# paolomandica/HALO

Measured on AMD Instinct MI355X. Metric: acquisition-scored images/sec (1024x2048, C=256, 19 cls), higher is better.
Workload: dtype f64

## Files before the change

halo_amd/_lib.py:

```python
import ctypes as C
import os
import threading

from . import _build

F32, F64 = 0, 1
I64, I32, U8 = 2, 3, 4
F16, BF16 = 5, 6
UNC = {"entropy": 0, "pixel_entropy": 1, "oracle_acc": 2}
UNC_ZEROS = 3
PUR = {"ripu": 0, "oracle_ripu": 1, "hyper": 2, "none": 3, "radius": 4, "euc_norm": 5}
E_UNSUPPORTED = -2
SELECT = {"auto": 0, "serial": 1, "binned": 2}
LOSS_CE, LOSS_NL = 1, 2
SWEEP_REASONS = ("done", "bad_values", "bin_overflow", "survivors", "exhausted", "not_run")
PAD = {"zeros": 0, "reflect": 1, "replicate": 2, "circular": 3}
FLAG_NORMALIZE = 1
WINDOW = {"box": 0, "hist": 1}
WINDOW_ROUTES = ("generic", "tile3", "tiled")


def score_flags(normalize, padding_mode="zeros"):
    return (FLAG_NORMALIZE if normalize else 0) | (PAD[padding_mode] << 8)

# ... 101 lines not shown
    "halo_sgd_plan": (_int, [C.POINTER(_i64), _i64, C.POINTER(_i64), C.POINTER(_i64), C.POINTER(_i64)]),
    "halo_sgd_step": (_int, [C.POINTER(SgdArgs), _vp]),
    "halo_event_create": (_vp, []),
    "halo_event_record": (_int, [_vp, _vp]),
    "halo_event_elapsed_ms": (_int, [_vp, _vp, C.POINTER(C.c_float)]),
    "halo_event_destroy": (_int, [_vp]),
    "halo_pack_pick_tables": (_int, [_vp, _vp, _i64, _i64, _vp, _i64, _vp]),
    "halo_reset_round_state": (_int, [_vp, _vp, _vp, _i64, _vp]),
    "halo_undo_picks": (_int, [_vp, _vp, _i64, _i64, _i64, _i64, _i64, _i64, _vp, _vp, _vp, _vp]),
    "halo_device_identity": (_int, [_int, C.c_char_p, _sz]),
    "halo_select_workspace_bytes": (_sz, [_i64, _i64, _i64, _i64, _i64]),
    "halo_score_range_bytes": (_sz, [_i64]),
    "halo_score_range": (_int, [_vp, _int, _i64, _i64, _i64, _vp, _vp]),
    "halo_greedy_select": (_int, [_vp, _int, _i64, _i64, _i64, _i64, _i64, _i64, _vp, _vp, _vp, _vp, _vp, _vp,
                                  _vp, _sz, _int, _vp, _vp, _vp]),
}

ABI_VERSION = 13

_lock = threading.Lock()
_handle = None


class HaloHipError(RuntimeError):
    pass


class HaloUnsupported(HaloHipError):
    """The kernel declined this configuration (HALO_E_UNSUPPORTED); the caller may take another HIP route."""

# ... 136 lines not shown
```

halo_amd/core/active/build.py:

```python
import math
import os
import struct
import zlib

import numpy as np
import torch
from PIL import Image

from ... import _lib
from ..configs import cfg
from ..utils.hyperbolic import HyperMapper, bilinear_align_corners
from .floating_region import FloatingRegionScore, new_score_range, score_maps, score_maps_lowres, _workspace


def greedy_select(score, n_regions, active_radius, mask_radius, active, selected, active_mask, ground_truth,
                  return_picks=True, method=None, out=None, score_range=None, handover=None):
    dev = _lib.require_device(score, active, selected, active_mask, ground_truth)
    B, H, W = score.shape
    for t in (score, active, selected, active_mask, ground_truth):
        assert t.shape == (B, H, W) and t.is_contiguous(), "greedy_select expects contiguous (B,H,W) tensors"
    assert active.dtype == torch.bool and selected.dtype == torch.bool
    assert active_mask.dtype == torch.int64 and ground_truth.dtype == torch.int64
    n = int(max(0, min(int(n_regions), H * W)))
    picks = n_picked = None
    if out is not None:
        picks, n_picked = out
        assert picks.shape == (B, max(n, 1), 3) and picks.dtype == torch.float64 and picks.is_contiguous() and picks.device == dev
        assert n_picked.shape == (B,) and n_picked.dtype == torch.int32 and n_picked.is_contiguous() and n_picked.device == dev
        return_picks = True
    elif return_picks:
        picks = torch.zeros((B, max(n, 1), 3), dtype=torch.float64, device=dev)
        n_picked = torch.zeros((B,), dtype=torch.int32, device=dev)
    if handover is not None:
        assert handover.shape == (B, 2) and handover.dtype == torch.int32 and handover.is_contiguous() and handover.device == dev
    if n == 0 or B == 0:
        if handover is not None:
            handover.zero_()
        return (picks[:, :0], n_picked) if return_picks else None
    L = _lib.lib()
    name = method or os.environ.get("HALO_SELECT", "auto")
    if name not in _lib.SELECT:
        raise ValueError("greedy_select: method must be one of %s, got %r" % (sorted(_lib.SELECT), name))
    method = _lib.SELECT[name]
    nws = L.halo_select_workspace_bytes(B, H, W, n, int(mask_radius)) if method != _lib.SELECT["serial"] else 256
    ws = _workspace(dev, nws, "select")
    if score_range is not None:
        assert score_range.is_contiguous() and score_range.device == dev and score_range.numel() >= L.halo_score_range_bytes(B)
    rc = L.halo_greedy_select(_lib.ptr(score), _lib.dtype_code(score), B, H, W, n, int(active_radius),
                              int(mask_radius), _lib.ptr(active), _lib.ptr(selected), _lib.ptr(active_mask),
                              _lib.ptr(ground_truth), _lib.ptr(picks), _lib.ptr(n_picked), _lib.ptr(ws), ws.numel(),
                              method, _lib.ptr(score_range), _lib.ptr(handover), _lib.stream_ptr(dev))
    _lib.check(rc, "halo_greedy_select")
    return (picks, n_picked) if return_picks else None


def _stage(t, dev, dtype):
    if t.device == dev and t.dtype == dtype and t.is_contiguous():
        return t, False
    return t.to(device=dev, dtype=dtype).contiguous(), True


def select_pixels_to_label(score, active_regions, active_radius, mask_radius, active, selected, active_mask,
                           ground_truth):
    dev = _lib.require_device(score)
    assert score.dim() == 2, "score must be (H, W)"
    sc, sc_c = _stage(score, dev, score.dtype if score.dtype in (torch.float32, torch.float64) else torch.float32)
    ac, ac_c = _stage(active, dev, torch.bool)
# ... 648 lines not shown
```

halo_amd/csrc/halo_select.hip:

```cpp
#include "halo_select_common.hpp"

namespace halo {

constexpr int SEL_TPB_MAIN = 512;
constexpr int SEL_TPB_RESUME = 256;

struct SelGeom { int H, W, th_shift, tw_shift, nty, ntx, nt; };

template <typename T, int TSH, int TSW>
__device__ __forceinline__ Cand tile_reduce(const T *__restrict__ sc, const SelGeom &g, int ty, int tx, int lane,
                                            int wy0, int wy1, int wx0, int wx1, int py0 = 1, int py1 = 0, int px0 = 1,
                                            int px1 = 0)
{
    constexpr int TW = 1 << TSW, NPL = (1 << (TSH + TSW)) / 64;
    static_assert(NPL >= 1, "tile smaller than a wave");
    const int x0 = tx << TSW, y0 = ty << TSH;
    double v[NPL];
#pragma unroll
    for (int i = 0; i < NPL; ++i) {
        const int e = lane + 64 * i;
        const int y = y0 + (e >> TSW), x = x0 + (e & (TW - 1));
        const int yc = y < g.H ? y : g.H - 1, xc = x < g.W ? x : g.W - 1;
        v[i] = (double)sc[(size_t)yc * g.W + xc];
    }
// ... 195 lines not shown
static bool serial_supported(int64_t H, int64_t W)
{
    if (H > 65535 || W > 65535) return false;
    const SelGeom g = make_geom(H, W);
    return (size_t)g.nt * 12 <= 96 * 1024;
}

extern "C" size_t halo_select_workspace_bytes(int64_t B, int64_t H, int64_t W, int64_t n_regions, int64_t mask_radius)
{
    if (B <= 0 || H <= 0 || W <= 0) return 0;
    if (n_regions > H * W) n_regions = H * W;
    const BinPlan p = binned_plan(B, H, W, n_regions, 0, mask_radius);
    return p.ok ? p.total_bytes + 256 : 256;
}

template <typename T, int A, int B_, int EPT>
static int launch_serial(const SelGeom &g, size_t lds, dim3 grid, hipStream_t st, void *score, int n_regions, int arad, int mrad,
                         uint8_t *active, uint8_t *selected, int64_t *active_mask, const int64_t *gt, double *picks,
                         int32_t *n_picked, const SelHdr *resume, int n_images)
{
    static LdsLimitSeen seen;
    if (lds > 64 * 1024 && !raise_lds_limit(seen, (const void *)k_greedy_select<T, A, B_, EPT>, 128 * 1024))
        return fail(HALO_E_LAUNCH, "halo_greedy_select: cannot raise the dynamic LDS limit");
    hipLaunchKernelGGL((k_greedy_select<T, A, B_, EPT>), grid, dim3(SEL_TPB_MAIN), lds, st, (T *)score, g, n_regions, arad, mrad, active,
                       selected, (long long *)active_mask, (const long long *)gt, picks, n_picked, resume, n_images);
    return HALO_OK;
}

template <typename T, int A, int B_, int EPT>
static int launch_resume(const SelGeom &g, size_t lds, dim3 grid, hipStream_t st, void *score, int n_regions, int arad, int mrad,
// ... 102 lines not shown
```

halo_amd/csrc/halo_select_binned.hip:

```cpp
#include <stdlib.h>
#include <string.h>

#include "halo_select_plan.hpp"

namespace halo {

constexpr int SW_TPB = 256;
constexpr int SW_SURV = 256;
constexpr int FWIN = 1024;

constexpr int BIN_CAP = 128;
constexpr int PL_U = 8;
constexpr int SW_MB = 4;

struct BinWs {
    SelHdr *hdr;
    SelHdr *rng;
    const unsigned *rng_hist;
    unsigned *hist1, *cbase, *cm;
    unsigned *fcur;
    unsigned long long *ckey;
    unsigned *cpos;
    unsigned long long *okmin_inv, *okmax;
    unsigned *plist;
// ... 75 lines not shown
            const unsigned long long k = order_key(v[u]);
            if (k < KEY_POS_INF && k != KEY_NEG_INF) {
                double t;
                atomicAdd(&h[coarse_bin(v[u], r, t)], 1u);
            }
        }
    }
    __syncthreads();
    unsigned *g = ws.hist1 + (size_t)b * NB1;
    for (int j = threadIdx.x; j < NB1; j += 256)
        if (h[j]) atomicAdd(&g[j], h[j]);
}

__global__ void __launch_bounds__(256) k_sel_scan1(BinWs ws, BinGeom g)
{
    __shared__ unsigned sc_c[256], sc_m[256], s_t1;
    const int b = blockIdx.x, tid = threadIdx.x;
    SelHdr *hdr = ws.hdr + b;
    const ValRange r = sel_range(ws.rng[b]);
    const bool ext = ws.rng_hist && (ws.rng[b].flags & SEL_F_HIST);
    const unsigned *hist = (ext ? ws.rng_hist : ws.hist1) + (size_t)b * NB1;
    unsigned c[8], m[8], tc = 0, tm = 0;
#pragma unroll
    for (int i = 0; i < 8; ++i) {
        c[i] = r.ok ? hist[tid * 8 + i] : 0u;
        m[i] = (c[i] + g.target - 1) / g.target;
        tc += c[i];
        tm += m[i];
    }
    sc_c[tid] = tc;
    sc_m[tid] = tm;
    if (tid == 0) s_t1 = 0;
    __syncthreads();
    for (int d = 1; d < 256; d <<= 1) {
        const unsigned ac = tid + d < 256 ? sc_c[tid + d] : 0u, am = tid + d < 256 ? sc_m[tid + d] : 0u;
        __syncthreads();
        sc_c[tid] += ac;
        sc_m[tid] += am;
        __syncthreads();
    }
    unsigned above_c = tid + 1 < 256 ? sc_c[tid + 1] : 0u, above_m = tid + 1 < 256 ? sc_m[tid + 1] : 0u;
    unsigned S[8], M[8];
#pragma unroll
    for (int i = 7; i >= 0; --i) {
        M[i] = above_m;
        above_c += c[i];
        above_m += m[i];
        S[i] = above_c;
    }
    int mine = -1;
#pragma unroll
    for (int i = 0; i < 8; ++i)
        if (S[i] >= g.kneed) mine = tid * 8 + i;
    if (mine > 0) atomicMax(&s_t1, (unsigned)mine);
    unsigned *cb = ws.cbase + (size_t)b * NB1, *cmm = ws.cm + (size_t)b * NB1;
#pragma unroll
    for (int i = 0; i < 8; ++i) { cb[tid * 8 + i] = M[i]; cmm[tid * 8 + i] = m[i]; }
    __syncthreads();
    unsigned t1 = s_t1;
    if ((int)(t1 >> 3) == tid) {
        const int i = t1 & 7;
        unsigned trunc = 0, nf;
        unsigned s_here = 0, m_here = 0, M_here = 0;
#pragma unroll
        for (int q = 0; q < 8; ++q)
            if (q == i) { s_here = S[q]; m_here = m[q]; M_here = M[q]; }
        if (!r.ok) { t1 = NB1; trunc = 1; nf = 0; }
        else if (s_here > g.captot) { t1 += 1; trunc = 1; nf = M_here; }
        else nf = M_here + m_here;
        if (ext && t1 > 0) trunc = 1;
        hdr->t1 = t1;
        hdr->truncated = trunc;
        hdr->nf = nf;
    }
    __syncthreads();
    if (ext && tid == 0) ws.rng[b].flags &= ~(unsigned)SEL_F_HIST;
}

template <typename T>
__global__ void __launch_bounds__(256) k_sel_place(const T *__restrict__ score, BinWs ws, BinGeom g)
{
    __shared__ unsigned s_base[NB1], s_m[NB1];
    const int b = blockIdx.y, tid = threadIdx.x;
    SelHdr *hdr = ws.hdr + b;
    const ValRange r = sel_range(ws.rng[b]);
    const unsigned t1 = hdr->t1;
    if (!r.ok || t1 >= NB1) return;
    for (int j = tid; j < NB1; j += 256) { s_base[j] = ws.cbase[(size_t)b * NB1 + j]; s_m[j] = ws.cm[(size_t)b * NB1 + j]; }
    __syncthreads();
    const T *sc = score + (size_t)b * g.H * g.W;
    unsigned *fcur = ws.fcur + (size_t)b * g.nfmax;
    unsigned long long *ckey = ws.ckey + (size_t)b * g.nfmax * BIN_CAP;
    unsigned *cpos = ws.cpos + (size_t)b * g.nfmax * BIN_CAP;
    bool overflow = false;
    for (int y = blockIdx.x; y < g.H; y += gridDim.x)
        for (int x0 = 0; x0 < g.W; x0 += PL_U * 256) {
            double v[PL_U];
#pragma unroll
            for (int u = 0; u < PL_U; ++u) {
                const int x = x0 + u * 256 + tid;
                v[u] = x < g.W ? (double)sc[(size_t)y * g.W + x] : __longlong_as_double(0xfff0000000000000ll);
            }
            unsigned long long k[PL_U];
            unsigned f[PL_U], slot[PL_U];
            bool cand[PL_U];
#pragma unroll
            for (int u = 0; u < PL_U; ++u) {
                k[u] = order_key(v[u]);
                cand[u] = k[u] < KEY_POS_INF && k[u] != KEY_NEG_INF;
                double t = 0.0;
                const int j = cand[u] ? coarse_bin(v[u], r, t) : 0;
                cand[u] = cand[u] && (unsigned)j >= t1;
                f[u] = 0;
                if (cand[u]) {
                    const unsigned mj = s_m[j];
                    unsigned sb = (unsigned)((t - (double)j) * (double)mj);
                    sb = sb > mj - 1 ? mj - 1 : sb;
                    f[u] = s_base[j] + (mj - 1 - sb);
                }
            }
            unsigned long long cm[PL_U];
            unsigned f_first = 0u, tot = 0u;
            cm[0] = __ballot(cand[0]);
            bool uni = __builtin_popcountll(cm[0]) >= 32;
            if (uni) {
                f_first = (unsigned)__builtin_amdgcn_readlane((int)f[0], (int)__builtin_ctzll(cm[0]));
                tot = (unsigned)__builtin_popcountll(cm[0]);
// ... 17 lines not shown
            }
#pragma unroll
            for (int u = 0; u < PL_U; ++u)
                if (cand[u]) {
                    if (slot[u] < (unsigned)BIN_CAP) {
                        const size_t sl = (size_t)f[u] * BIN_CAP + slot[u];
                        ckey[sl] = k[u];
                        cpos[sl] = ((unsigned)(x0 + u * 256 + tid) << 16) | (unsigned)y;
                    } else overflow = true;
                }
        }
    if (__any(overflow) && (tid & 63) == 0) atomicOr(&hdr->flags, (unsigned)SEL_F_OVERFLOW);
}

template <typename T>
__global__ void __launch_bounds__(256) k_sel_full_extrema(const T *__restrict__ score, BinWs ws, BinGeom g)
{
    __shared__ unsigned s_base[NB1], s_m[NB1];
    const int b = blockIdx.y, tid = threadIdx.x;
    const SelHdr *hdr = ws.hdr + b;
    if (!(hdr->flags & SEL_F_OVERFLOW)) return;
    const ValRange r = sel_range(ws.rng[b]);
    const unsigned t1 = hdr->t1;
    if (!r.ok || t1 >= NB1) return;
    for (int j = tid; j < NB1; j += 256) { s_base[j] = ws.cbase[(size_t)b * NB1 + j]; s_m[j] = ws.cm[(size_t)b * NB1 + j]; }
    __syncthreads();
    const T *sc = score + (size_t)b * g.H * g.W;
    const unsigned *fcur = ws.fcur + (size_t)b * g.nfmax;
    unsigned long long *okmin_inv = ws.okmin_inv + (size_t)b * g.nfmax, *okmax = ws.okmax + (size_t)b * g.nfmax;
    for (int y = blockIdx.x; y < g.H; y += gridDim.x)
        for (int x0 = 0; x0 < g.W; x0 += 256) {
            const int x = x0 + tid;
            const double v = x < g.W ? (double)sc[(size_t)y * g.W + x] : __longlong_as_double(0xfff0000000000000ll);
            const unsigned long long k = order_key(v);
            bool cand = k < KEY_POS_INF && k != KEY_NEG_INF;
            double t = 0.0;
            const int j = cand ? coarse_bin(v, r, t) : 0;
            cand = cand && (unsigned)j >= t1;
            unsigned f = 0;
            if (cand) {
                const unsigned mj = s_m[j];
                unsigned sb = (unsigned)((t - (double)j) * (double)mj);
                sb = sb > mj - 1 ? mj - 1 : sb;
                f = s_base[j] + (mj - 1 - sb);
            }
            const bool full = cand && fcur[f] > (unsigned)BIN_CAP;
            unsigned long long todo = __ballot(full);
            while (todo) {
                const int l0 = (int)__builtin_ctzll(todo);
                const unsigned f0 = (unsigned)__builtin_amdgcn_readlane((int)f, l0);
                const bool mine = full && f == f0;
                const unsigned long long kx = wave_max_u64(mine ? k : 0ull), kn = wave_max_u64(mine ? ~k : 0ull);
                if ((tid & 63) == l0) { atomicMax(&okmax[f0], kx); atomicMax(&okmin_inv[f0], kn); }
// ... 94 lines not shown
        if (__ballot(undecided) == 0ull) break;
    }
    const bool is_pick = alive && ((pickm >> lane) & 1ull) != 0ull;
    const int idx = np + (int)__builtin_popcountll(before & pickm);
    if (is_pick && idx < g.n_regions) {
        plist[idx] = pos;
        const int pcx = (int)__umulhi((unsigned)x, g.cmul), pcy = (int)__umulhi((unsigned)y, g.cmul);
        grid[(pcy + 1) * g.gstride + pcx + 1] = (unsigned char)(1 + (((y - pcy * cs) << 4) | (x - pcx * cs)));
    }
    np += (int)__builtin_popcountll(pickm);
    if (np >= g.n_regions) { np = g.n_regions; return 1; }
    return 0;
}

__global__ void __launch_bounds__(SW_TPB, 5) k_sel_sweep(BinWs ws, BinGeom g, int *__restrict__ n_picked, const void *__restrict__ score_maps,
                                                      int score_f64)
{
    extern __shared__ __attribute__((aligned(16))) unsigned char smem[];
    unsigned char *grid = smem;
    unsigned *gridw = reinterpret_cast<unsigned *>(smem);
    unsigned long long *skey = reinterpret_cast<unsigned long long *>(smem + g.grid_bytes);
    unsigned *spos = reinterpret_cast<unsigned *>(skey + SW_SURV);
    unsigned *fwin = spos + SW_SURV;
    unsigned *ctl = fwin + FWIN + 1;

    __builtin_amdgcn_s_setprio(3);
    const int b = blockIdx.x, tid = threadIdx.x, lane = tid & 63, wave = tid >> 6;
    SelHdr *hdr = ws.hdr + b;
    const unsigned nf = hdr->nf;
    const bool truncated = hdr->truncated != 0;
    const unsigned *fcnt = ws.fcur + (size_t)b * g.nfmax;
    const unsigned long long *ckey = ws.ckey + (size_t)b * g.nfmax * BIN_CAP;
    const unsigned *cpos = ws.cpos + (size_t)b * g.nfmax * BIN_CAP;
    unsigned *plist = ws.plist + (size_t)b * g.n_regions;
    const unsigned long long *okmin_inv = ws.okmin_inv + (size_t)b * g.nfmax, *okmax = ws.okmax + (size_t)b * g.nfmax;
    const double *map64 = score_f64 ? (const double *)score_maps + (size_t)b * g.H * g.W : nullptr;
    const float *map32 = score_f64 ? nullptr : (const float *)score_maps + (size_t)b * g.H * g.W;

    for (unsigned i = tid * 16; i < g.grid_bytes; i += SW_TPB * 16) *reinterpret_cast<uint4 *>(smem + i) = make_uint4(0, 0, 0, 0);
    if (tid == 0) { ctl[0] = 0; ctl[1] = 0; }
    __syncthreads();

    int np = 0;
    int fin = 0;
    int why = HALO_SWEEP_DONE;
    const int r = g.mrad, cs = g.cs;

    struct Chunk { unsigned start[SW_MB], cnt[SW_MB], total; bool last, valid, plateau; unsigned pbin; };
    unsigned fw0 = 0, fwn = 0;
    unsigned it_f = 0;
    auto next_chunk = [&]() {
        Chunk c;
#pragma unroll
        for (int i = 0; i < SW_MB; ++i) { c.start[i] = 0; c.cnt[i] = 0; }
        c.total = 0; c.last = true; c.valid = false; c.plateau = false; c.pbin = 0;
        int nb = 0;
        while (it_f < nf) {
            if (fwn == 0 || it_f >= fw0 + fwn) {
                lds_barrier();
                fw0 = it_f;
                fwn = nf - it_f < (unsigned)FWIN ? nf - it_f : (unsigned)FWIN;
                for (unsigned i = tid; i < fwn; i += SW_TPB) fwin[i] = fcnt[fw0 + i];
                __syncthreads();
            }
            const unsigned n = fwin[it_f - fw0];
// ... 150 lines not shown
            if (fin) break;
            knext = wave_max_u64(knext);
            lds_barrier();
            if (lane == 0) skey[wave] = knext;
            lds_barrier();
            knext = skey[0];
#pragma unroll
            for (int i = 1; i < SW_TPB / 64; ++i) knext = skey[i] > knext ? skey[i] : knext;
            lds_barrier();
            if (knext == 0ull) break;
            K = knext;
        }
    };
    auto step = [&](const Chunk &c, const Regs &d) {
        if (c.plateau) { plateau_scan(c.pbin); return; }
        push((unsigned)tid < c.total && grid_alive(d.pos), d.key, d.pos);
        if (!c.last) return;
        resolve_listed();
    };
    Chunk c0 = next_chunk(), c1, c2;
    Regs d0, d1, d2;
    issue(c0, d0);
    c1 = next_chunk(); issue(c1, d1);
    c2 = next_chunk(); issue(c2, d2);
    while (true) {
        if (!c0.valid || fin) break;
        step(c0, d0);
        c0 = next_chunk(); issue(c0, d0);
        if (!c1.valid || fin) break;
        step(c1, d1);
        c1 = next_chunk(); issue(c1, d1);
        if (!c2.valid || fin) break;
        step(c2, d2);
        c2 = next_chunk(); issue(c2, d2);
    }
#ifdef HALO_SWEEP_STAMPS
    if (tid == 0) {
        hdr->pad[0] = (unsigned)(t_f >> 4); hdr->pad[1] = (unsigned)(t_a >> 4); hdr->pad[2] = (unsigned)(t_r >> 4); hdr->pad[3] = (unsigned)(t_b >> 4);
        hdr->nvalid = (unsigned)nb; hdr->ncand = (unsigned)t_surv; hdr->flags = (unsigned)t_smax;
    }
#endif
    if (tid == 0) {
        if (fin == 0) {
            fin = truncated ? 2 : 1;
            if (truncated) why = hdr->t1 >= (unsigned)NB1 ? HALO_SWEEP_BAD_VALUES : HALO_SWEEP_EXHAUSTED;
        }
        if (ws.handover) { ws.handover[2 * b] = fin == 1 ? HALO_SWEEP_DONE : why; ws.handover[2 * b + 1] = np; }
        hdr->np = np;
        hdr->status = fin == 1 ? SEL_DONE : SEL_BAIL;
        if (fin == 1 && n_picked) n_picked[b] = np;
    }
}

constexpr int APPLY_WGS = 32;

template <typename T>
__global__ void __launch_bounds__(256) k_sel_apply(T *__restrict__ score, unsigned char *__restrict__ active,
                                                   unsigned char *__restrict__ selected, long long *__restrict__ active_mask,
                                                   const long long *__restrict__ gt, double *__restrict__ picks, BinWs ws, BinGeom g)
{
    const int b = blockIdx.y, lane = threadIdx.x & 63;
    const int np = ws.hdr[b].np;
    const size_t hw = (size_t)g.H * g.W;
    T *sc = score + (size_t)b * hw;
    unsigned char *act = active + (size_t)b * hw, *sel = selected + (size_t)b * hw;
// ... 21 lines not shown
        const int aw = ax1 - ax0 + 1, an = aw * (ay1 - ay0 + 1);
        const int mw = mx1 - mx0 + 1, mn = mw * (my1 - my0 + 1);
        for (int e = lane; e < an; e += 64) {
            const size_t o = (size_t)(ay0 + e / aw) * g.W + (ax0 + e % aw);
            sel[o] = 1;
            am[o] = gtb[o];
        }
        for (int e = lane; e < mn; e += 64) {
            const size_t o = (size_t)(my0 + e / mw) * g.W + (mx0 + e % mw);
            sc[o] = neg_inf;
            act[o] = 1;
        }
    }
}

}

using namespace halo;

namespace halo {

BinPlan binned_plan(int64_t B, int64_t H, int64_t W, int64_t n_regions, int64_t arad, int64_t mrad)
{
    BinPlan p;
    memset(&p, 0, sizeof(p));
    if (B <= 0 || H <= 0 || W <= 0 || n_regions <= 0 || H > 65535 || W > 65535 || mrad < 1 || mrad > 14) return p;
    BinGeom &g = p.g;
    g.H = (int)H; g.W = (int)W; g.n_regions = (int)n_regions; g.arad = (int)arad; g.mrad = (int)mrad;
    g.cs = (int)mrad + 1;
    g.gcy = (int)cdiv(H, g.cs);
    g.gcx = (int)cdiv(W, g.cs);
    g.gstride = (int)align_up((size_t)g.gcx + 2, 4);
    g.cmul = (unsigned)((0x100000000ull + (unsigned)g.cs - 1) / (unsigned)g.cs);
    g.grid_bytes = (unsigned)align_up((size_t)(g.gcy + 2) * g.gstride + 8, 16);
    p.lds_bytes = g.grid_bytes + (size_t)SW_SURV * 12 + (FWIN + 1) * 4 + 16;
    if (p.lds_bytes > 156 * 1024) return p;
    const unsigned long long hw = (unsigned long long)H * W, win = (unsigned long long)(2 * mrad + 1) * (2 * mrad + 1);
    const unsigned long long kneed = win * (unsigned long long)n_regions < hw ? win * (unsigned long long)n_regions : hw;
    unsigned long long cap = 2 * kneed < 65536 ? 65536 : 2 * kneed;
    if (cap > hw) cap = hw;
    g.kneed = (unsigned)kneed;
    g.captot = (unsigned)cap;
    g.target = (unsigned)(BIN_CAP / 2);
    g.nfmax = (unsigned)(cap / g.target + NB1 + 1);
    size_t o = 0;
    auto take = [&](size_t per_image) { const size_t at = o; o += align_up(per_image * (size_t)B, 256); return at; };
    p.off_hdr = take(sizeof(SelHdr));
    p.off_hist1 = take((size_t)NB1 * 4);
    p.off_fcur = take((size_t)g.nfmax * 4);
    p.off_okmin = take((size_t)g.nfmax * 8);
    p.off_okmax = take((size_t)g.nfmax * 8);
    p.zero_bytes = o;
    p.off_cbase = take((size_t)NB1 * 4);
    p.off_cm = take((size_t)NB1 * 4);
    p.off_ckey = take((size_t)g.nfmax * BIN_CAP * 8);
    p.off_cpos = take((size_t)g.nfmax * BIN_CAP * 4);
// ... 12 lines not shown
    ws.rng = ws.hdr;
    const unsigned gx = (unsigned)(cdiv(hw, 256) < 128 ? cdiv(hw, 256) : 128);
    if (dtype == HALO_F64) hipLaunchKernelGGL(k_sel_range<double>, dim3(gx, (unsigned)B), dim3(256), 0, st, (const double *)score, (long long)hw, ws);
    else hipLaunchKernelGGL(k_sel_range<float>, dim3(gx, (unsigned)B), dim3(256), 0, st, (const float *)score, (long long)hw, ws);
    return HALO_OK;
}

int binned_select(void *score, int dtype, int64_t B, const BinPlan &p, uint8_t *active, uint8_t *selected, int64_t *active_mask,
                  const int64_t *gt, double *picks, int32_t *n_picked, void *workspace, size_t workspace_bytes, hipStream_t st,
                  SelHdr **hdr_out, const void *score_range, int32_t *handover)
{
    if (!workspace || workspace_bytes < p.total_bytes) return fail(HALO_E_WORKSPACE, "halo_greedy_select: workspace too small");
    char *base = (char *)(((uintptr_t)workspace + 255) & ~(uintptr_t)255);
    if ((size_t)(base - (char *)workspace) + p.total_bytes - 256 > workspace_bytes) return fail(HALO_E_WORKSPACE, "halo_greedy_select: workspace too small");
    BinWs ws;
    ws.hdr = (SelHdr *)(base + p.off_hdr);
    ws.rng = score_range ? (SelHdr *)score_range : ws.hdr;
    ws.rng_hist = score_range ? (const unsigned *)((const char *)score_range + range_hist_offset(B)) : nullptr;
    ws.hist1 = (unsigned *)(base + p.off_hist1);
    ws.fcur = (unsigned *)(base + p.off_fcur);
    ws.okmin_inv = (unsigned long long *)(base + p.off_okmin);
    ws.okmax = (unsigned long long *)(base + p.off_okmax);
    ws.cbase = (unsigned *)(base + p.off_cbase);
    ws.cm = (unsigned *)(base + p.off_cm);
    ws.ckey = (unsigned long long *)(base + p.off_ckey);
    ws.cpos = (unsigned *)(base + p.off_cpos);
    ws.plist = (unsigned *)(base + p.off_plist);
    ws.handover = handover;
    const BinGeom &g = p.g;
    const long long hw = (long long)g.H * g.W;
// ... 1 lines not shown
        const size_t n16 = p.zero_bytes / 16;
        const unsigned gz = (unsigned)(cdiv((int64_t)n16, 256) < 512 ? cdiv((int64_t)n16, 256) : 512);
        hipLaunchKernelGGL(k_sel_zero, dim3(gz ? gz : 1u), dim3(256), 0, st, (uint4 *)base, n16);
    }
    const unsigned gx = (unsigned)(cdiv(hw, 256) < 128 ? cdiv(hw, 256) : 128);
    const unsigned gy = (unsigned)(g.H < 128 ? g.H : 128);
    dim3 blk(256);
    if (dtype == HALO_F64) {
        if (!score_range) hipLaunchKernelGGL(k_sel_range<double>, dim3(gx, (unsigned)B), blk, 0, st, (const double *)score, hw, ws);
        hipLaunchKernelGGL(k_sel_hist1<double>, dim3(gx, (unsigned)B), blk, 0, st, (const double *)score, hw, ws);
    } else {
        if (!score_range) hipLaunchKernelGGL(k_sel_range<float>, dim3(gx, (unsigned)B), blk, 0, st, (const float *)score, hw, ws);
        hipLaunchKernelGGL(k_sel_hist1<float>, dim3(gx, (unsigned)B), blk, 0, st, (const float *)score, hw, ws);
    }
    hipLaunchKernelGGL(k_sel_scan1, dim3((unsigned)B), blk, 0, st, ws, g);
    if (dtype == HALO_F64) hipLaunchKernelGGL(k_sel_place<double>, dim3(gy, (unsigned)B), blk, 0, st, (const double *)score, ws, g);
    else hipLaunchKernelGGL(k_sel_place<float>, dim3(gy, (unsigned)B), blk, 0, st, (const float *)score, ws, g);
    {
        const dim3 ge((unsigned)(g.H < 64 ? g.H : 64), (unsigned)B);
        if (dtype == HALO_F64) hipLaunchKernelGGL(k_sel_full_extrema<double>, ge, blk, 0, st, (const double *)score, ws, g);
        else hipLaunchKernelGGL(k_sel_full_extrema<float>, ge, blk, 0, st, (const float *)score, ws, g);
    }
    static LdsLimitSeen seen;
    if (!raise_lds_limit(seen, (const void *)k_sel_sweep, 160 * 1024))
        return fail(HALO_E_LAUNCH, "halo_greedy_select: cannot raise the dynamic LDS limit");
    hipLaunchKernelGGL(k_sel_sweep, dim3((unsigned)B), dim3(SW_TPB), p.lds_bytes, st, ws, g, n_picked, (const void *)score, dtype == HALO_F64 ? 1 : 0);
    const dim3 ga((unsigned)(cdiv(g.n_regions, 4) < APPLY_WGS ? cdiv(g.n_regions, 4) : APPLY_WGS), (unsigned)B);
    if (dtype == HALO_F64)
        hipLaunchKernelGGL(k_sel_apply<double>, ga, blk, 0, st, (double *)score, active, selected, (long long *)active_mask, (const long long *)gt, picks, ws, g);
    else
        hipLaunchKernelGGL(k_sel_apply<float>, ga, blk, 0, st, (float *)score, active, selected, (long long *)active_mask, (const long long *)gt, picks, ws, g);
    *hdr_out = ws.hdr;
    return check_launch("halo_greedy_select (binned)");
}

}
```

halo_amd/csrc/halo_select_common.hpp:

```cpp
#pragma once
#include "halo_common.hpp"

namespace halo {

constexpr unsigned long long KEY_NAN = 0xffffffffffffffffull;
constexpr unsigned long long KEY_NEG_INF = 0x000fffffffffffffull;
constexpr unsigned long long KEY_POS_INF = 0xfff0000000000000ull;

__device__ __forceinline__ unsigned long long order_key(double v)
{
    const bool isnan = v != v;
    v = v == 0.0 ? 0.0 : v;
    const unsigned long long u = (unsigned long long)__double_as_longlong(v);
    const unsigned long long k = (u >> 63) ? ~u : (u | 0x8000000000000000ull);
    return isnan ? KEY_NAN : k;
}
__device__ __forceinline__ double key_value(unsigned long long k)
{
    if (k == KEY_NAN) return __longlong_as_double(0x7ff8000000000000ll);
    const unsigned long long u = (k >> 63) ? (k & 0x7fffffffffffffffull) : ~k;
    return __longlong_as_double((long long)u);
}

struct Cand { unsigned long long key; unsigned pos; };
// ... 33 lines not shown
}

__device__ __forceinline__ void lds_barrier() { asm volatile("s_waitcnt lgkmcnt(0)\n\ts_barrier" ::: "memory"); }

struct SelHdr {
    unsigned long long kmin_inv;
    unsigned long long kmax;
    unsigned nvalid;
    unsigned flags;
    unsigned ncand;
    unsigned nf;
    unsigned t1;
    unsigned truncated;
    int status;
    int np;
    unsigned pad[4];
};
static_assert(sizeof(SelHdr) == 64, "SelHdr is 64 bytes");
enum { SEL_RUN = 0, SEL_DONE = 1, SEL_BAIL = 2 };
enum { SEL_F_BAD = 1,
       SEL_F_OVERFLOW = 2,
       SEL_F_HIST = 4 };

constexpr int NB1 = 2048;

__host__ __device__ inline size_t range_hist_offset(long long B) { return ((size_t)B * sizeof(SelHdr) + 255) / 256 * 256; }

struct ValRange { double lo, scale; bool ok; };

__device__ __forceinline__ ValRange sel_range(const SelHdr &h)
{
    ValRange r;
    const double lo = key_value(~h.kmin_inv), hi = key_value(h.kmax);
    r.lo = lo;
// ... 15 lines not shown
```

halo_amd/csrc/halo_select_plan.hpp:

```cpp
#pragma once
#include "halo_select_common.hpp"

namespace halo {

struct BinGeom {
    int H, W, n_regions, arad, mrad;
    unsigned kneed, captot, target, nfmax;
    int cs, gcy, gcx, gstride;
    unsigned cmul;
    unsigned grid_bytes;
};

struct BinPlan {
    bool ok;
    BinGeom g;
    size_t zero_bytes, total_bytes, lds_bytes;
    size_t off_hdr, off_hist1, off_fcur, off_okmin, off_okmax, off_cbase, off_cm, off_ckey, off_cpos, off_plist;
};

BinPlan binned_plan(int64_t B, int64_t H, int64_t W, int64_t n_regions, int64_t arad, int64_t mrad);

int binned_select(void *score, int dtype, int64_t B, const BinPlan &p, uint8_t *active, uint8_t *selected, int64_t *active_mask,
                  const int64_t *gt, double *picks, int32_t *n_picked, void *workspace, size_t workspace_bytes, hipStream_t st,
                  SelHdr **hdr_out, const void *score_range = nullptr, int32_t *handover = nullptr);

int score_range_exact(const void *score, int dtype, int64_t B, int64_t hw, void *range_out, hipStream_t st);

}
```

include/halo_hip.h:

```cpp
#ifndef HALO_HIP_H
#define HALO_HIP_H

#include <stddef.h>
#include <stdint.h>

#ifdef __cplusplus
extern "C" {
#endif

#define HALO_ABI_VERSION 13

enum { HALO_F32 = 0, HALO_F64 = 1, HALO_I64 = 2, HALO_I32 = 3, HALO_U8 = 4, HALO_F16 = 5, HALO_BF16 = 6 };

enum { HALO_OK = 0, HALO_E_ARG = -1, HALO_E_UNSUPPORTED = -2, HALO_E_WORKSPACE = -3, HALO_E_LAUNCH = -4 };

enum { HALO_UNC_ENTROPY = 0, HALO_UNC_PIXEL_ENTROPY = 1, HALO_UNC_ORACLE_ACC = 2, HALO_UNC_ZEROS = 3 };

enum { HALO_PAD_ZEROS = 0, HALO_PAD_REFLECT = 1, HALO_PAD_REPLICATE = 2, HALO_PAD_CIRCULAR = 3 };
enum { HALO_FLAG_NORMALIZE = 1 };
#define HALO_FLAG_PAD(mode) ((mode) << 8)

enum { HALO_PUR_RIPU = 0, HALO_PUR_ORACLE_RIPU = 1, HALO_PUR_HYPER = 2, HALO_PUR_NONE = 3,
       HALO_PUR_RADIUS = 4, HALO_PUR_EUC_NORM = 5 };

// ... 82 lines not shown
enum { HALO_SELECT_AUTO = 0, HALO_SELECT_SERIAL = 1, HALO_SELECT_BINNED = 2 };
size_t halo_select_workspace_bytes(int64_t B, int64_t H, int64_t W, int64_t n_regions, int64_t mask_radius);
enum { HALO_SWEEP_DONE = 0,
       HALO_SWEEP_BAD_VALUES = 1,
       HALO_SWEEP_BIN_OVERFLOW = 2,
       HALO_SWEEP_SURVIVORS = 3,
       HALO_SWEEP_EXHAUSTED = 4,
       HALO_SWEEP_NOT_RUN = 5 };
size_t halo_score_range_bytes(int64_t B);
int halo_score_range(const void *score, int dtype, int64_t B, int64_t H, int64_t W, void *score_range, void *stream);
int halo_greedy_select(void *score, int dtype, int64_t B, int64_t H, int64_t W, int64_t n_regions,
                       int64_t active_radius, int64_t mask_radius, uint8_t *active, uint8_t *selected,
                       int64_t *active_mask, const int64_t *gt, double *picks, int32_t *n_picked,
                       void *workspace, size_t workspace_bytes, int method, const void *score_range,
                       int32_t *handover, void *stream);

int halo_pack_pick_tables(const double *picks, const int32_t *n_picked, int64_t B, int64_t n_regions, int32_t *wire,
                          int64_t wire_row_stride, void *stream);
int halo_reset_round_state(uint8_t *active, uint8_t *selected, int64_t *active_mask, int64_t n_pixels, void *stream);
int halo_undo_picks(const double *picks, const int32_t *n_picked, int64_t B, int64_t H, int64_t W, int64_t n_regions,
                    int64_t active_radius, int64_t mask_radius, uint8_t *active, uint8_t *selected, int64_t *active_mask,
                    void *stream);
int halo_device_identity(int device, char *buf, size_t len);

size_t halo_loss_workspace_bytes(int64_t n);
int halo_negative_learning_fwd(const float *p, int64_t n, double threshold, double *sums, void *workspace,
                               size_t workspace_bytes, void *stream);
int halo_negative_learning_bwd(const float *p, int64_t n, double threshold, const double *sums, const float *gloss,
                               float *gp, void *stream);
int halo_local_consistent_fwd(const float *x, const int64_t *label, int64_t B, int64_t O, int64_t h, int64_t w, int kl,
// ... 138 lines not shown
```

Baseline: 1403.

## Split binned greedy selection into a small first tranche with fallback round

The binned greedy selector now places and sweeps only the top tranche of candidates first, sized at 16x n_regions instead of the full window-times-regions budget. A second, smaller-grid place/extrema/sweep round runs only when the first tranche did not finish selection, resuming from the saved picks. This is meant to cut candidate placement and sweep work in the common case, at the cost of extra kernel launches and a second pass when the tranche runs dry. A stats query kernel is also added for diagnostics.

After: 1427 (median of 6 runs). 1.7% higher.

```diff
diff --git a/halo_amd/_lib.py b/halo_amd/_lib.py
--- a/halo_amd/_lib.py
+++ b/halo_amd/_lib.py
@@ -139,6 +139,8 @@
     "halo_score_range": (_int, [_vp, _int, _i64, _i64, _i64, _vp, _vp]),
     "halo_greedy_select": (_int, [_vp, _int, _i64, _i64, _i64, _i64, _i64, _i64, _vp, _vp, _vp, _vp, _vp, _vp,
                                   _vp, _sz, _int, _vp, _vp, _vp]),
+    "halo_select_first_tranche": (_i64, [_i64, _i64, _i64, _i64]),
+    "halo_select_stats": (_int, [_vp, _sz, _i64, _i64, _i64, _i64, _i64, _vp, _vp]),
 }
 
 ABI_VERSION = 13
diff --git a/halo_amd/core/active/build.py b/halo_amd/core/active/build.py
--- a/halo_amd/core/active/build.py
+++ b/halo_amd/core/active/build.py
@@ -14,7 +14,7 @@
 
 
 def greedy_select(score, n_regions, active_radius, mask_radius, active, selected, active_mask, ground_truth,
-                  return_picks=True, method=None, out=None, score_range=None, handover=None):
+                  return_picks=True, method=None, out=None, score_range=None, handover=None, stats=None):
     dev = _lib.require_device(score, active, selected, active_mask, ground_truth)
     B, H, W = score.shape
     for t in (score, active, selected, active_mask, ground_truth):
@@ -33,9 +33,13 @@
         n_picked = torch.zeros((B,), dtype=torch.int32, device=dev)
     if handover is not None:
         assert handover.shape == (B, 2) and handover.dtype == torch.int32 and handover.is_contiguous() and handover.device == dev
+    if stats is not None:
+        assert stats.shape == (B, 3) and stats.dtype == torch.int32 and stats.is_contiguous() and stats.device == dev
     if n == 0 or B == 0:
         if handover is not None:
             handover.zero_()
+        if stats is not None:
+            stats.zero_()
         return (picks[:, :0], n_picked) if return_picks else None
     L = _lib.lib()
     name = method or os.environ.get("HALO_SELECT", "auto")
@@ -51,6 +55,12 @@
                               _lib.ptr(ground_truth), _lib.ptr(picks), _lib.ptr(n_picked), _lib.ptr(ws), ws.numel(),
                               method, _lib.ptr(score_range), _lib.ptr(handover), _lib.stream_ptr(dev))
     _lib.check(rc, "halo_greedy_select")
+    if stats is not None:
+        if method == _lib.SELECT["serial"]:
+            stats.zero_()
+        else:
+            _lib.check(L.halo_select_stats(_lib.ptr(ws), ws.numel(), B, H, W, n, int(mask_radius), _lib.ptr(stats), _lib.stream_ptr(dev)),
+                       "halo_select_stats")
     return (picks, n_picked) if return_picks else None
 
 
diff --git a/halo_amd/csrc/halo_select.hip b/halo_amd/csrc/halo_select.hip
--- a/halo_amd/csrc/halo_select.hip
+++ b/halo_amd/csrc/halo_select.hip
@@ -233,6 +233,24 @@
     return p.ok ? p.total_bytes + 256 : 256;
 }
 
+extern "C" int64_t halo_select_first_tranche(int64_t H, int64_t W, int64_t n_regions, int64_t mask_radius)
+{
+    if (H <= 0 || W <= 0 || n_regions <= 0 || mask_radius < 0) return 0;
+    if (n_regions > H * W) n_regions = H * W;
+    const unsigned long long hw = (unsigned long long)H * W, win = (unsigned long long)(2 * mask_radius + 1) * (2 * mask_radius + 1);
+    const unsigned long long kneed = win * (unsigned long long)n_regions < hw ? win * (unsigned long long)n_regions : hw;
+    return (int64_t)tranche_first(kneed, (unsigned long long)n_regions);
+}
+
+extern "C" int halo_select_stats(const void *workspace, size_t workspace_bytes, int64_t B, int64_t H, int64_t W, int64_t n_regions,
+                                 int64_t mask_radius, int32_t *stats, void *stream)
+{
+    if (!stats || B <= 0 || H <= 0 || W <= 0 || n_regions < 0 || mask_radius < 0) return fail(HALO_E_ARG, "halo_select_stats: null/empty argument");
+    if (n_regions > H * W) n_regions = H * W;
+    const BinPlan p = binned_plan(B, H, W, n_regions, 0, mask_radius);
+    return binned_stats(B, p, workspace, workspace_bytes, stats, (hipStream_t)stream);
+}
+
 template <typename T, int A, int B_, int EPT>
 static int launch_serial(const SelGeom &g, size_t lds, dim3 grid, hipStream_t st, void *score, int n_regions, int arad, int mrad,
                          uint8_t *active, uint8_t *selected, int64_t *active_mask, const int64_t *gt, double *picks,
diff --git a/halo_amd/csrc/halo_select_binned.hip b/halo_amd/csrc/halo_select_binned.hip
--- a/halo_amd/csrc/halo_select_binned.hip
+++ b/halo_amd/csrc/halo_select_binned.hip
@@ -113,7 +113,7 @@
 
 __global__ void __launch_bounds__(256) k_sel_scan1(BinWs ws, BinGeom g)
 {
-    __shared__ unsigned sc_c[256], sc_m[256], s_t1;
+    __shared__ unsigned sc_c[256], sc_m[256], s_t1, s_t1a, s_nfa;
     const int b = blockIdx.x, tid = threadIdx.x;
     SelHdr *hdr = ws.hdr + b;
     const ValRange r = sel_range(ws.rng[b]);
@@ -129,7 +129,7 @@
     }
     sc_c[tid] = tc;
     sc_m[tid] = tm;
-    if (tid == 0) s_t1 = 0;
+    if (tid == 0) { s_t1 = 0; s_t1a = 0; s_nfa = 0; }
     __syncthreads();
     for (int d = 1; d < 256; d <<= 1) {
         const unsigned ac = tid + d < 256 ? sc_c[tid + d] : 0u, am = tid + d < 256 ? sc_m[tid + d] : 0u;
@@ -152,11 +152,23 @@
     for (int i = 0; i < 8; ++i)
         if (S[i] >= g.kneed) mine = tid * 8 + i;
     if (mine > 0) atomicMax(&s_t1, (unsigned)mine);
+    int mine_a = -1;
+#pragma unroll
+    for (int i = 0; i < 8; ++i)
+        if (S[i] >= g.kfirst) mine_a = tid * 8 + i;
+    if (mine_a > 0) atomicMax(&s_t1a, (unsigned)mine_a);
     unsigned *cb = ws.cbase + (size_t)b * NB1, *cmm = ws.cm + (size_t)b * NB1;
 #pragma unroll
     for (int i = 0; i < 8; ++i) { cb[tid * 8 + i] = M[i]; cmm[tid * 8 + i] = m[i]; }
     __syncthreads();
     unsigned t1 = s_t1;
+    const unsigned t1a_raw = s_t1a;
+    if ((int)(t1a_raw >> 3) == tid) {
+#pragma unroll
+        for (int q = 0; q < 8; ++q)
+            if (q == (int)(t1a_raw & 7)) s_nfa = M[q] + m[q];
+    }
+    __syncthreads();
     if ((int)(t1 >> 3) == tid) {
         const int i = t1 & 7;
         unsigned trunc = 0, nf;
@@ -171,20 +183,24 @@
         hdr->t1 = t1;
         hdr->truncated = trunc;
         hdr->nf = nf;
+        const bool one = !r.ok || t1a_raw < t1;
+        hdr->t1a = one ? t1 : t1a_raw;
+        hdr->nf_a = one ? nf : s_nfa;
     }
     __syncthreads();
     if (ext && tid == 0) ws.rng[b].flags &= ~(unsigned)SEL_F_HIST;
 }
 
 template <typename T>
-__global__ void __launch_bounds__(256) k_sel_place(const T *__restrict__ score, BinWs ws, BinGeom g)
+__global__ void __launch_bounds__(256) k_sel_place(const T *__restrict__ score, BinWs ws, BinGeom g, int round)
 {
     __shared__ unsigned s_base[NB1], s_m[NB1];
     const int b = blockIdx.y, tid = threadIdx.x;
     SelHdr *hdr = ws.hdr + b;
+    if (round != 0 && hdr->status != SEL_MORE) return;
     const ValRange r = sel_range(ws.rng[b]);
-    const unsigned t1 = hdr->t1;
-    if (!r.ok || t1 >= NB1) return;
+    const unsigned t1 = round == 0 ? hdr->t1a : hdr->t1, t_end = round == 0 ? (unsigned)NB1 : hdr->t1a;
+    if (!r.ok || t1 >= t_end) return;
     for (int j = tid; j < NB1; j += 256) { s_base[j] = ws.cbase[(size_t)b * NB1 + j]; s_m[j] = ws.cm[(size_t)b * NB1 + j]; }
     __syncthreads();
     const T *sc = score + (size_t)b * g.H * g.W;
@@ -209,7 +225,7 @@
                 cand[u] = k[u] < KEY_POS_INF && k[u] != KEY_NEG_INF;
                 double t = 0.0;
                 const int j = cand[u] ? coarse_bin(v[u], r, t) : 0;
-                cand[u] = cand[u] && (unsigned)j >= t1;
+                cand[u] = cand[u] && (unsigned)j - t1 < t_end - t1;
                 f[u] = 0;
                 if (cand[u]) {
                     const unsigned mj = s_m[j];
@@ -257,15 +273,16 @@
 }
 
 template <typename T>
-__global__ void __launch_bounds__(256) k_sel_full_extrema(const T *__restrict__ score, BinWs ws, BinGeom g)
+__global__ void __launch_bounds__(256) k_sel_full_extrema(const T *__restrict__ score, BinWs ws, BinGeom g, int round)
 {
     __shared__ unsigned s_base[NB1], s_m[NB1];
     const int b = blockIdx.y, tid = threadIdx.x;
     const SelHdr *hdr = ws.hdr + b;
     if (!(hdr->flags & SEL_F_OVERFLOW)) return;
+    if (round != 0 && hdr->status != SEL_MORE) return;
     const ValRange r = sel_range(ws.rng[b]);
-    const unsigned t1 = hdr->t1;
-    if (!r.ok || t1 >= NB1) return;
+    const unsigned t1 = round == 0 ? hdr->t1a : hdr->t1, t_end = round == 0 ? (unsigned)NB1 : hdr->t1a;
+    if (!r.ok || t1 >= t_end) return;
     for (int j = tid; j < NB1; j += 256) { s_base[j] = ws.cbase[(size_t)b * NB1 + j]; s_m[j] = ws.cm[(size_t)b * NB1 + j]; }
     __syncthreads();
     const T *sc = score + (size_t)b * g.H * g.W;
@@ -279,7 +296,7 @@
             bool cand = k < KEY_POS_INF && k != KEY_NEG_INF;
             double t = 0.0;
             const int j = cand ? coarse_bin(v, r, t) : 0;
-            cand = cand && (unsigned)j >= t1;
+            cand = cand && (unsigned)j - t1 < t_end - t1;
             unsigned f = 0;
             if (cand) {
                 const unsigned mj = s_m[j];
@@ -404,7 +421,7 @@
 }
 
 __global__ void __launch_bounds__(SW_TPB, 5) k_sel_sweep(BinWs ws, BinGeom g, int *__restrict__ n_picked, const void *__restrict__ score_maps,
-                                                      int score_f64)
+                                                      int score_f64, int round)
 {
     extern __shared__ __attribute__((aligned(16))) unsigned char smem[];
     unsigned char *grid = smem;
@@ -417,7 +434,8 @@
     __builtin_amdgcn_s_setprio(3);
     const int b = blockIdx.x, tid = threadIdx.x, lane = tid & 63, wave = tid >> 6;
     SelHdr *hdr = ws.hdr + b;
-    const unsigned nf = hdr->nf;
+    if (round != 0 && hdr->status != SEL_MORE) return;
+    const unsigned nf = round == 0 ? hdr->nf_a : hdr->nf;
     const bool truncated = hdr->truncated != 0;
     const unsigned *fcnt = ws.fcur + (size_t)b * g.nfmax;
     const unsigned long long *ckey = ws.ckey + (size_t)b * g.nfmax * BIN_CAP;
@@ -432,13 +450,24 @@
     __syncthreads();
 
     int np = 0;
+    if (round != 0) {
+        np = hdr->np;
+        for (int i = tid; i < np; i += SW_TPB) {
+            const unsigned pos = plist[i];
+            const int px = (int)(pos >> 16), py = (int)(pos & 0xffffu);
+            const int pcx = (int)__umulhi((unsigned)px, g.cmul), pcy = (int)__umulhi((unsigned)py, g.cmul);
+            grid[(pcy + 1) * g.gstride + pcx + 1] = (unsigned char)(1 + (((py - pcy * g.cs) << 4) | (px - pcx * g.cs)));
+        }
+        __syncthreads();
+    }
+    unsigned consumed = 0;
     int fin = 0;
     int why = HALO_SWEEP_DONE;
     const int r = g.mrad, cs = g.cs;
 
     struct Chunk { unsigned start[SW_MB], cnt[SW_MB], total; bool last, valid, plateau; unsigned pbin; };
     unsigned fw0 = 0, fwn = 0;
-    unsigned it_f = 0;
+    unsigned it_f = round == 0 ? 0u : hdr->nf_a;
     auto next_chunk = [&]() {
         Chunk c;
 #pragma unroll
@@ -619,6 +648,7 @@
     };
     auto step = [&](const Chunk &c, const Regs &d) {
         if (c.plateau) { plateau_scan(c.pbin); return; }
+        consumed += c.total;
         push((unsigned)tid < c.total && grid_alive(d.pos), d.key, d.pos);
         if (!c.last) return;
         resolve_listed();
@@ -639,21 +669,24 @@
         step(c2, d2);
         c2 = next_chunk(); issue(c2, d2);
     }
+    if (tid == 0) {
+        hdr->consumed = (round == 0 ? 0u : hdr->consumed) + consumed;
+        hdr->rounds = (unsigned)round + 1u;
+        hdr->np = np;
+        if (fin == 0 && round == 0 && hdr->t1a != hdr->t1) hdr->status = SEL_MORE;
+        else {
+            if (fin == 0) {
+                fin = truncated ? 2 : 1;
+                if (truncated) why = hdr->t1 >= (unsigned)NB1 ? HALO_SWEEP_BAD_VALUES : HALO_SWEEP_EXHAUSTED;
+            }
+            if (ws.handover) { ws.handover[2 * b] = fin == 1 ? HALO_SWEEP_DONE : why; ws.handover[2 * b + 1] = np; }
+            hdr->status = fin == 1 ? SEL_DONE : SEL_BAIL;
+            if (fin == 1 && n_picked) n_picked[b] = np;
 #ifdef HALO_SWEEP_STAMPS
-    if (tid == 0) {
-        hdr->pad[0] = (unsigned)(t_f >> 4); hdr->pad[1] = (unsigned)(t_a >> 4); hdr->pad[2] = (unsigned)(t_r >> 4); hdr->pad[3] = (unsigned)(t_b >> 4);
-        hdr->nvalid = (unsigned)nb; hdr->ncand = (unsigned)t_surv; hdr->flags = (unsigned)t_smax;
-    }
+            hdr->t1a = (unsigned)(t_f >> 4); hdr->nf_a = (unsigned)(t_a >> 4); hdr->consumed = (unsigned)(t_r >> 4); hdr->rounds = (unsigned)(t_b >> 4);
+            hdr->nvalid = (unsigned)nb; hdr->ncand = (unsigned)t_surv; hdr->flags = (unsigned)t_smax;
 #endif
-    if (tid == 0) {
-        if (fin == 0) {
-            fin = truncated ? 2 : 1;
-            if (truncated) why = hdr->t1 >= (unsigned)NB1 ? HALO_SWEEP_BAD_VALUES : HALO_SWEEP_EXHAUSTED;
-        }
-        if (ws.handover) { ws.handover[2 * b] = fin == 1 ? HALO_SWEEP_DONE : why; ws.handover[2 * b + 1] = np; }
-        hdr->np = np;
-        hdr->status = fin == 1 ? SEL_DONE : SEL_BAIL;
-        if (fin == 1 && n_picked) n_picked[b] = np;
+        }
     }
 }
 
@@ -705,6 +738,30 @@
     }
 }
 
+__global__ void __launch_bounds__(256) k_sel_stats(BinWs ws, BinGeom g, int *__restrict__ stats)
+{
+    __shared__ unsigned s_sum[4];
+    const int b = blockIdx.x, tid = threadIdx.x;
+    if (!ws.hdr) {
+        if (tid < 3) stats[3 * b + tid] = 0;
+        return;
+    }
+    const SelHdr *hdr = ws.hdr + b;
+    const unsigned nf = hdr->rounds ? hdr->nf : 0u;
+    const unsigned *fcnt = ws.fcur + (size_t)b * g.nfmax;
+    unsigned n = 0;
+    for (unsigned f = tid; f < nf; f += 256) n += fcnt[f] < (unsigned)BIN_CAP ? fcnt[f] : (unsigned)BIN_CAP;
+#pragma unroll
+    for (int o = 32; o > 0; o >>= 1) n += __shfl_xor(n, o, 64);
+    if ((tid & 63) == 0) s_sum[tid >> 6] = n;
+    __syncthreads();
+    if (tid == 0) {
+        stats[3 * b] = (int)(s_sum[0] + s_sum[1] + s_sum[2] + s_sum[3]);
+        stats[3 * b + 1] = (int)hdr->consumed;
+        stats[3 * b + 2] = (int)hdr->rounds;
+    }
+}
+
 }
 
 using namespace halo;
@@ -731,6 +788,7 @@
     unsigned long long cap = 2 * kneed < 65536 ? 65536 : 2 * kneed;
     if (cap > hw) cap = hw;
     g.kneed = (unsigned)kneed;
+    g.kfirst = (unsigned)tranche_first(kneed, (unsigned long long)n_regions);
     g.captot = (unsigned)cap;
     g.target = (unsigned)(BIN_CAP / 2);
     g.nfmax = (unsigned)(cap / g.target + NB1 + 1);
@@ -773,6 +831,7 @@
     char *base = (char *)(((uintptr_t)workspace + 255) & ~(uintptr_t)255);
     if ((size_t)(base - (char *)workspace) + p.total_bytes - 256 > workspace_bytes) return fail(HALO_E_WORKSPACE, "halo_greedy_select: workspace too small");
     BinWs ws;
+    memset(&ws, 0, sizeof(ws));
     ws.hdr = (SelHdr *)(base + p.off_hdr);
     ws.rng = score_range ? (SelHdr *)score_range : ws.hdr;
     ws.rng_hist = score_range ? (const unsigned *)((const char *)score_range + range_hist_offset(B)) : nullptr;
@@ -804,17 +863,22 @@
         hipLaunchKernelGGL(k_sel_hist1<float>, dim3(gx, (unsigned)B), blk, 0, st, (const float *)score, hw, ws);
     }
     hipLaunchKernelGGL(k_sel_scan1, dim3((unsigned)B), blk, 0, st, ws, g);
-    if (dtype == HALO_F64) hipLaunchKernelGGL(k_sel_place<double>, dim3(gy, (unsigned)B), blk, 0, st, (const double *)score, ws, g);
-    else hipLaunchKernelGGL(k_sel_place<float>, dim3(gy, (unsigned)B), blk, 0, st, (const float *)score, ws, g);
-    {
-        const dim3 ge((unsigned)(g.H < 64 ? g.H : 64), (unsigned)B);
-        if (dtype == HALO_F64) hipLaunchKernelGGL(k_sel_full_extrema<double>, ge, blk, 0, st, (const double *)score, ws, g);
-        else hipLaunchKernelGGL(k_sel_full_extrema<float>, ge, blk, 0, st, (const float *)score, ws, g);
-    }
     static LdsLimitSeen seen;
     if (!raise_lds_limit(seen, (const void *)k_sel_sweep, 160 * 1024))
         return fail(HALO_E_LAUNCH, "halo_greedy_select: cannot raise the dynamic LDS limit");
-    hipLaunchKernelGGL(k_sel_sweep, dim3((unsigned)B), dim3(SW_TPB), p.lds_bytes, st, ws, g, n_picked, (const void *)score, dtype == HALO_F64 ? 1 : 0);
+    for (int round = 0; round < 2; ++round) {
+        const unsigned gp = round == 0 ? gy : (gy + 3) / 4;
+        if (dtype == HALO_F64) hipLaunchKernelGGL(k_sel_place<double>, dim3(gp, (unsigned)B), blk, 0, st, (const double *)score, ws, g, round);
+        else hipLaunchKernelGGL(k_sel_place<float>, dim3(gp, (unsigned)B), blk, 0, st, (const float *)score, ws, g, round);
+        {
+            const unsigned gh = (unsigned)(g.H < 64 ? g.H : 64);
+            const dim3 ge(round == 0 ? gh : (gh + 3) / 4, (unsigned)B);
+            if (dtype == HALO_F64) hipLaunchKernelGGL(k_sel_full_extrema<double>, ge, blk, 0, st, (const double *)score, ws, g, round);
+            else hipLaunchKernelGGL(k_sel_full_extrema<float>, ge, blk, 0, st, (const float *)score, ws, g, round);
+        }
+        hipLaunchKernelGGL(k_sel_sweep, dim3((unsigned)B), dim3(SW_TPB), p.lds_bytes, st, ws, g, n_picked, (const void *)score,
+                           dtype == HALO_F64 ? 1 : 0, round);
+    }
     const dim3 ga((unsigned)(cdiv(g.n_regions, 4) < APPLY_WGS ? cdiv(g.n_regions, 4) : APPLY_WGS), (unsigned)B);
     if (dtype == HALO_F64)
         hipLaunchKernelGGL(k_sel_apply<double>, ga, blk, 0, st, (double *)score, active, selected, (long long *)active_mask, (const long long *)gt, picks, ws, g);
@@ -824,4 +888,19 @@
     return check_launch("halo_greedy_select (binned)");
 }
 
-}
+int binned_stats(int64_t B, const BinPlan &p, const void *workspace, size_t workspace_bytes, int32_t *stats, hipStream_t st)
+{
+    BinWs ws;
+    memset(&ws, 0, sizeof(ws));
+    if (p.ok) {
+        if (!workspace || workspace_bytes < p.total_bytes) return fail(HALO_E_WORKSPACE, "halo_select_stats: workspace too small");
+        char *base = (char *)(((uintptr_t)workspace + 255) & ~(uintptr_t)255);
+        if ((size_t)(base - (char *)workspace) + p.total_bytes - 256 > workspace_bytes) return fail(HALO_E_WORKSPACE, "halo_select_stats: workspace too small");
+        ws.hdr = (SelHdr *)(base + p.off_hdr);
+        ws.fcur = (unsigned *)(base + p.off_fcur);
+    }
+    hipLaunchKernelGGL(k_sel_stats, dim3((unsigned)B), dim3(256), 0, st, ws, p.g, stats);
+    return check_launch("halo_select_stats");
+}
+
+}
diff --git a/halo_amd/csrc/halo_select_common.hpp b/halo_amd/csrc/halo_select_common.hpp
--- a/halo_amd/csrc/halo_select_common.hpp
+++ b/halo_amd/csrc/halo_select_common.hpp
@@ -71,10 +71,14 @@
     unsigned truncated;
     int status;
     int np;
-    unsigned pad[4];
+    unsigned t1a;
+    unsigned nf_a;
+    unsigned consumed;
+    unsigned rounds;
 };
 static_assert(sizeof(SelHdr) == 64, "SelHdr is 64 bytes");
-enum { SEL_RUN = 0, SEL_DONE = 1, SEL_BAIL = 2 };
+enum { SEL_RUN = 0, SEL_DONE = 1, SEL_BAIL = 2,
+       SEL_MORE = 3 };
 enum { SEL_F_BAD = 1,
        SEL_F_OVERFLOW = 2,
        SEL_F_HIST = 4 };
diff --git a/halo_amd/csrc/halo_select_plan.hpp b/halo_amd/csrc/halo_select_plan.hpp
--- a/halo_amd/csrc/halo_select_plan.hpp
+++ b/halo_amd/csrc/halo_select_plan.hpp
@@ -3,9 +3,16 @@
 
 namespace halo {
 
+constexpr unsigned TRANCHE_F = 16;
+
+inline unsigned long long tranche_first(unsigned long long kneed, unsigned long long n_regions)
+{
+    return kneed < n_regions * TRANCHE_F ? kneed : n_regions * TRANCHE_F;
+}
+
 struct BinGeom {
     int H, W, n_regions, arad, mrad;
-    unsigned kneed, captot, target, nfmax;
+    unsigned kneed, kfirst, captot, target, nfmax;
     int cs, gcy, gcx, gstride;
     unsigned cmul;
     unsigned grid_bytes;
@@ -24,6 +31,8 @@
                   const int64_t *gt, double *picks, int32_t *n_picked, void *workspace, size_t workspace_bytes, hipStream_t st,
                   SelHdr **hdr_out, const void *score_range = nullptr, int32_t *handover = nullptr);
 
+int binned_stats(int64_t B, const BinPlan &p, const void *workspace, size_t workspace_bytes, int32_t *stats, hipStream_t st);
+
 int score_range_exact(const void *score, int dtype, int64_t B, int64_t hw, void *range_out, hipStream_t st);
 
 }
diff --git a/include/halo_hip.h b/include/halo_hip.h
--- a/include/halo_hip.h
+++ b/include/halo_hip.h
@@ -120,6 +120,9 @@
                        int64_t *active_mask, const int64_t *gt, double *picks, int32_t *n_picked,
                        void *workspace, size_t workspace_bytes, int method, const void *score_range,
                        int32_t *handover, void *stream);
+int64_t halo_select_first_tranche(int64_t H, int64_t W, int64_t n_regions, int64_t mask_radius);
+int halo_select_stats(const void *workspace, size_t workspace_bytes, int64_t B, int64_t H, int64_t W, int64_t n_regions,
+                      int64_t mask_radius, int32_t *stats, void *stream);
 
 int halo_pack_pick_tables(const double *picks, const int32_t *n_picked, int64_t B, int64_t n_regions, int32_t *wire,
                           int64_t wire_row_stride, void *stream);
```
